# lab-cosmo/torch-pme

Hardware: AMD Instinct MI355X
Metric: atom-steps/sec (energy+forces) (higher is better)
Workload: dtype f32

## Files before the change

### include/mipme.h

```cpp
#ifndef MIPME_H
#define MIPME_H

#include <stdint.h>

#ifdef __cplusplus
extern "C" {
#endif

#define MIPME_VERSION 408

enum { MIPME_F32 = 0, MIPME_F64 = 1 };
enum { MIPME_I64 = 0, MIPME_I32 = 1 };
enum { MIPME_LAGRANGE = 0, MIPME_P3M = 1 };
enum { MIPME_COULOMB = 0, MIPME_INVERSE_POWER_LAW = 1 };

enum {
  MIPME_OK = 0,
  MIPME_EINVAL = -1,
  MIPME_EHIP = -2,
  MIPME_EFFT = -3,
  MIPME_EUNSUPPORTED = -4
};

typedef struct {
// ... 233 lines not shown
  const mipme_potential_t* pot;
  int64_t n_atoms;
  const void* positions;
  const void* charges;
  const void* grad_out;
  const void* G;
  const void* phi_mesh;
  const void* rho_hat;
  const void* rho_dc;
  const void* phi_atoms;
  void* psi_mesh;
  void* psi_hat;
  void* hat_work;
  void* chi_mesh;
  void* dc;
  void* partials;
  void* grad_positions;
  void* grad_charges;
  void* grad_cell;
  void* atom_bins;
  const void* grad_scale;
  const void* mesh_field;
  int64_t kgrid_blocks_ready;
  const void* G_deriv;
} mipme_kspace_backward_args_t;
int mipme_kspace_backward(const mipme_kspace_backward_args_t* args);
int64_t mipme_cellgrad_partials_size(const mipme_mesh_t* mesh, int64_t n_atoms);

int64_t mipme_atom_bins_bytes(const mipme_mesh_t* mesh, int64_t n_atoms, int dtype);
const char* mipme_last_cosched_kernel(void);
int mipme_last_slot_fill(void);
int mipme_last_cell_riders(void);
int mipme_last_gather_pairs(void);
int mipme_plane_spread_parts(const mipme_mesh_t* mesh, int64_t n_atoms, int dtype);

int mipme_profile_enable(int on);
int64_t mipme_profile_report(char* buf, int64_t buflen);

int mipme_slab_forward(void* stream, int dtype, int axis, const mipme_mesh_t* mesh, double prefactor, int64_t n_atoms,
                       const void* positions, const void* charges, void* moments, void* pot);
int mipme_slab_backward(void* stream, int dtype, int axis, const mipme_mesh_t* mesh, double prefactor, int64_t n_atoms,
                        const void* positions, const void* charges, const void* grad_out, void* moments,
                        void* grad_positions, void* grad_charges, void* grad_cell);


int mipme_rspace_forward(void* stream, int dtype, int idx_dtype, int64_t n_pairs, int64_t n_atoms, int n_channels,
                         const void* pairs, const void* dist, const void* charges, const void* pair_mask,
                         int full_list, const mipme_potential_t* pot, int accumulate, void* out_pot);

int mipme_rspace_backward(void* stream, int dtype, int idx_dtype, int64_t n_pairs, int64_t n_atoms, int n_channels,
                          const void* pairs, const void* dist, const void* charges, const void* pair_mask,
                          int full_list, const mipme_potential_t* pot, const void* grad_out, const void* grad_scale,
                          void* grad_dist, void* grad_charges);

int mipme_dot_forward(void* stream, int dtype, int64_t n, const void* a, const void* b, void* scratch ,
                      void* out);
int mipme_dot_backward(void* stream, int dtype, int64_t n, const void* grad, const void* a, const void* b, void* grad_a,
                       void* grad_b);

int mipme_energy_log_push(void* stream, int dtype, int n, const void* src, void* log, void* cursor, int capacity);
int mipme_frames_table_energy_log(int dtype, int n_frames, void* host_table, int64_t host_table_bytes, void* log, void* cursors,
                                  int capacity);

int mipme_scaled_match(void* stream, int dtype, int64_t n, const void* g, const void* q, void* result, void* host_flag);
int64_t mipme_scaled_match_work(int64_t n);
int mipme_scaled_match_wide(void* stream, int dtype, int64_t n, const void* g, const void* q, void* result, void* host_flag,
// ... 357 lines not shown
```

### torch-pme_amd/_lib.py

```python

from __future__ import annotations

import ctypes as C
import os

import torch

_HERE = os.path.dirname(os.path.abspath(__file__))
LIB_PATH = os.environ.get("MIPME_LIB", os.path.join(_HERE, "libmipme.so"))

F32, F64 = 0, 1
I64, I32 = 0, 1
LAGRANGE, P3M = 0, 1
COULOMB, INVERSE_POWER_LAW = 0, 1

EXPORTS = (
    "mipme_last_error", "mipme_version", "mipme_fft_plan_create", "mipme_fft_plan_destroy", "mipme_kfilter_build",
    "mipme_convolve", "mipme_spread", "mipme_gather", "mipme_kspace_forward", "mipme_kspace_backward",
    "mipme_cellgrad_partials_size", "mipme_slab_forward", "mipme_slab_backward", "mipme_rspace_forward",
    "mipme_rspace_backward", "mipme_pair_distance_forward", "mipme_pair_distance_backward",
    "mipme_pair_partials_size", "mipme_topology_workspace_bytes", "mipme_topology_build", "mipme_topology_pack_shifts",
    "mipme_rspace_rows", "mipme_rspace_rows_value_bytes", "mipme_rspace_rows_tabulate", "mipme_rspace_rows_tabulated", "mipme_pair_distance_backward_rows", "mipme_rows_partials_size", "mipme_atom_bins_bytes", "mipme_plane_spread_parts", "mipme_last_cosched_kernel", "mipme_last_slot_fill", "mipme_last_cell_riders", "mipme_last_gather_pairs", "mipme_frames_counter_ints",
    "mipme_profile_enable", "mipme_profile_report", "mipme_dot_forward", "mipme_dot_backward", "mipme_energy_log_push", "mipme_frames_table_energy_log",
    "mipme_nl_workspace_bytes", "mipme_nl_bin", "mipme_nl_count", "mipme_nl_fill", "mipme_nl_stream",
    "mipme_topology_pack_entries", "mipme_sr_rows_fused", "mipme_sr_rows_finalize",
    "mipme_pack_pair_shifts", "mipme_pair_distance_forward_packed", "mipme_fft_plan_xfused", "mipme_fft_plan_kgrid_blocks", "mipme_fft_r2c",
    "mipme_ewald_filter", "mipme_ewald_structure", "mipme_ewald_potential", "mipme_ewald_backward",
    "mipme_frames_table_bytes", "mipme_frames_table_build", "mipme_frames_forward", "mipme_frames_backward",
    "mipme_frames_cell_work", "mipme_frames_table_contract", "mipme_frames_step",
    "mipme_frames_slab_work", "mipme_frames_table_slab", "mipme_frames_slab_step",
    "mipme_frames_table_cells", "mipme_frames_cells", "mipme_frames_cell_geometry",
    "mipme_scaled_match", "mipme_scaled_match_work", "mipme_scaled_match_wide", "mipme_md_supported", "mipme_md_lists_ints", "mipme_md_rebin", "mipme_md_step", "mipme_set_skip_flag", "mipme_energy_select", "mipme_energy_select_sum", "mipme_energy_select_contract",
    "mipme_kfilter_build_deriv", "mipme_cell_tail_work", "mipme_values_equal", "mipme_checksum", "mipme_checksum_words",
    "mipme_spread_jet", "mipme_gather_jet", "mipme_gather_jet3", "mipme_pair_sum", "mipme_pair_sum_rows", "mipme_pair_dot", "mipme_pair_diff", "mipme_pair_scatter",
    "mipme_dipole_rspace_forward", "mipme_dipole_rspace_backward", "mipme_dipole_partials_size", "mipme_dipole_structure",
    "mipme_dipole_field", "mipme_dipole_backward",
    "mipme_spline_eval", "mipme_spline_eval_reciprocal", "mipme_spline_kfilter_build",
    "mipme_combined_sr_eval", "mipme_combined_kfilter_build",
    "mipme_combined_step", "mipme_combined_step_work",
    "mipme_dipole_step", "mipme_dipole_step_work",
    "mipme_ewald_step", "mipme_ewald_step_work",
    "mipme_ewald_batch", "mipme_ewald_batch_work", "mipme_ewald_batch_table_bytes", "mipme_ewald_batch_table_build",
)


class PotentialDesc(C.Structure):
    _fields_ = [
        ("kind", C.c_int32),
        ("exponent", C.c_int32),
        ("smearing", C.c_double),
        ("prefactor", C.c_double),
        ("exclusion_radius", C.c_double),
        ("exclusion_degree", C.c_int32),
        ("_pad", C.c_int32),
    ]
# ... 443 lines not shown
        "mipme_checksum": [vp, vp, i64, vp, vp, vp],
        "mipme_energy_select": [vp, ci, i64, vp, vp, vp, vp, ci, vp, vp],
        "mipme_energy_select_sum": [vp, ci, i64, vp, vp, vp, vp, ci, vp, vp, vp],
        "mipme_energy_select_contract": [vp, ci, i64, vp, vp, vp, vp, ci, vp, vp, vp],
        "mipme_md_rebin": [C.POINTER(MdArgs)],
        "mipme_md_step": [C.POINTER(MdArgs)],
    }
    for name, argtypes in sig.items():
        fn = getattr(lib, name)
        fn.restype = ci
        fn.argtypes = argtypes
    lib.mipme_cellgrad_partials_size.restype = i64
    lib.mipme_cellgrad_partials_size.argtypes = [MP, i64]
    lib.mipme_dipole_partials_size.restype = i64
    lib.mipme_dipole_partials_size.argtypes = [i64, i64]
    lib.mipme_pair_partials_size.restype = i64
    lib.mipme_pair_partials_size.argtypes = [i64]
    lib.mipme_topology_workspace_bytes.restype = i64
    lib.mipme_topology_workspace_bytes.argtypes = [i64]
    lib.mipme_rows_partials_size.restype = i64
    lib.mipme_rows_partials_size.argtypes = [i64]
    lib.mipme_atom_bins_bytes.restype = i64
    lib.mipme_atom_bins_bytes.argtypes = [MP, i64, ci]
    lib.mipme_last_cosched_kernel.restype = C.c_char_p
    lib.mipme_last_cosched_kernel.argtypes = []
    if hasattr(lib, "mipme_last_slot_fill"):
        lib.mipme_last_slot_fill.restype = ci
        lib.mipme_last_slot_fill.argtypes = []
        lib.mipme_last_cell_riders.restype = ci
        lib.mipme_last_cell_riders.argtypes = []
    if hasattr(lib, "mipme_last_gather_pairs"):
        lib.mipme_last_gather_pairs.restype = ci
        lib.mipme_last_gather_pairs.argtypes = []
    lib.mipme_plane_spread_parts.restype = ci
    lib.mipme_plane_spread_parts.argtypes = [MP, i64, ci]
    lib.mipme_frames_counter_ints.restype = i64
    lib.mipme_frames_counter_ints.argtypes = [MP, i64, ci]
    lib.mipme_md_supported.restype = ci
    lib.mipme_md_supported.argtypes = [MP, PP, i64, ci]
    lib.mipme_md_lists_ints.restype = i64
    lib.mipme_md_lists_ints.argtypes = [MP, i64]
    lib.mipme_nl_workspace_bytes.restype = i64
    lib.mipme_nl_workspace_bytes.argtypes = [C.POINTER(NlDesc), i64]
    lib.mipme_rspace_rows_value_bytes.restype = i64
    lib.mipme_rspace_rows_value_bytes.argtypes = [ci, i64]
    lib.mipme_checksum_words.restype = i64
    lib.mipme_checksum_words.argtypes = []
    lib.mipme_cell_tail_work.restype = i64
    lib.mipme_cell_tail_work.argtypes = [vp, MP, i64]
    lib.mipme_fft_plan_xfused.restype = ci
    lib.mipme_fft_plan_xfused.argtypes = [vp]
    lib.mipme_fft_plan_kgrid_blocks.restype = i64
    lib.mipme_fft_plan_kgrid_blocks.argtypes = [vp]
    lib.mipme_frames_cell_work.restype = i64
    lib.mipme_frames_cell_work.argtypes = [MP, i64]
    lib.mipme_combined_step_work.restype = i64
    lib.mipme_combined_step_work.argtypes = [vp, MP, i64, ci]
    lib.mipme_dipole_step_work.restype = i64
    lib.mipme_dipole_step_work.argtypes = [i64, i64, ci]
    lib.mipme_ewald_step_work.restype = i64
    lib.mipme_ewald_step_work.argtypes = [i64, i64, ci]
    lib.mipme_ewald_batch_work.restype = i64
    lib.mipme_ewald_batch_work.argtypes = [ci, vp, vp, ci]
    lib.mipme_ewald_batch_table_bytes.restype = i64
    lib.mipme_ewald_batch_table_bytes.argtypes = [ci, vp, vp, ci]
    lib.mipme_frames_slab_work.restype = i64
# ... 136 lines not shown
```

### torch-pme_amd/csrc/api.hip

```cpp
#include <dlfcn.h>

#include <cmath>
#include <cstring>
#include <map>
#include <string>
#include <vector>

#include "host.h"

namespace mipme {

static thread_local char g_error[512] = "";

static thread_local const char* g_last_cosched = "";
void note_cosched_kernel(const char* name) { g_last_cosched = name ? name : ""; }
static thread_local int g_last_slot_fill = 0;
void note_slot_fill(int rider_atoms) { g_last_slot_fill = rider_atoms; }
static thread_local int g_last_cell_riders = 0;
void note_cell_riders(int n) { g_last_cell_riders = n; }
static thread_local int g_last_gather_pairs = 0;
void note_gather_pairs(int paired) { g_last_gather_pairs = paired; }
void set_error(const char* fmt, ...) {
  va_list ap;
  va_start(ap, fmt);
  vsnprintf(g_error, sizeof(g_error), fmt, ap);
  va_end(ap);
}

struct ProfEntry {
  const char* name;
  hipEvent_t a, b;
  int reps;
};
static constexpr int kProfRepeat = 8;
static bool g_prof_on = false;
static std::vector<ProfEntry> g_prof;

struct Roctx {
  int (*push)(const char*) = nullptr;
  int (*pop)() = nullptr;
  bool on = false;
  Roctx() {
    const char* e = getenv("MIPME_ROCTX");
    if (!e || e[0] == '0') return;
    for (const char* name : {"librocprofiler-sdk-roctx.so", "libroctx64.so"}) {
      if (void* h = dlopen(name, RTLD_NOW | RTLD_GLOBAL)) {
        push = (int (*)(const char*))dlsym(h, "roctxRangePushA");
        pop = (int (*)())dlsym(h, "roctxRangePop");
        if (push && pop) {
          on = true;
          return;
        }
      }
    }
// ... 839 lines not shown
  const ConvCell cc{a.G_deriv, cw.cwave, cw.n_waves, cw.wbuf, cw.rows, int(cw.n_riders), nullptr, nullptr, nullptr, nullptr};
  STAGE(st, "convolve_xfused", convolve_xfused(a.plan, st, a.rho_mesh, a.G, a.hat_work, a.phi_mesh, a.dc, 0, m, a.pot, nullptr,
                                               const_cast<void*>(tail.epart_k), sr_part, n_sr_part, nullptr, a.nan_flag,
                                               a.grad_cell ? &cc : nullptr));
  STAGE(st, "gather+energy+forces",
        live_gather<T>(st, m, a.n_atoms, a.records, a.atom_bins, a.live_lists, a.phi_mesh, a.dc, self_c, bg_c, a.potentials, nullptr,
                       &tail, a.nan_flag));
  if (a.grad_cell)
    STAGE(st, "cell_finalize",
          cell_tail_finalize_impl<T>(st, m, bg_c, 0.5, cw.n_riders, cw.n_bricks, cw.rows, cw.rpart, a.dc,
                                     a.aux_seed ? a.aux_seed : a.grad_seed, a.grad_cell, &tail));
  return MIPME_OK;
}


template <typename T>
static int scaled_match_wide_t(hipStream_t st, int64_t n, const void* g, const void* q, void* result, void* host_flag, void* work) {
  const int64_t nb = (n + 1024 * kMatchRegs - 1) / (1024 * kMatchRegs);
  MIPME_REQUIRE(nb < (int64_t(1) << 24), "mipme_scaled_match_wide: too many values");
  scaled_match_small_kernel<T, true><<<unsigned(nb), 1024, 0, st>>>(n, (const T*)g, (const T*)q, nullptr, nullptr, (double*)work);
  MIPME_LAUNCH_CHECK();
  scaled_match_combine_kernel<T><<<1, 256, 0, st>>>(int(nb), (const double*)work, (T*)result, (int*)host_flag);
  MIPME_LAUNCH_CHECK();
  return MIPME_OK;
}

extern "C" {

const char* mipme_last_error(void) { return g_error; }
const char* mipme_last_cosched_kernel(void) { return g_last_cosched; }
int mipme_last_slot_fill(void) { return g_last_slot_fill; }
int mipme_last_gather_pairs(void) { return g_last_gather_pairs; }
int mipme_last_cell_riders(void) { return g_last_cell_riders; }
int mipme_version(void) { return MIPME_VERSION; }

int mipme_fft_plan_create(int dtype, int nx, int ny, int nz, int batch, mipme_fft_plan** out) {
  return fft_plan_create(dtype, nx, ny, nz, batch, out);
}
int mipme_fft_plan_destroy(mipme_fft_plan* plan) { return fft_plan_destroy(plan); }

int mipme_kfilter_build(void* stream, int dtype, const mipme_mesh_t* mesh, const mipme_potential_t* pot, void* G) {
  int rc = validate_mesh(mesh);
  if (rc) return rc;
  MIPME_REQUIRE(G != nullptr, "G is NULL");
  hipStream_t st = (hipStream_t)stream;
  DT_SWITCH(dtype, kfilter_build_impl<float>(st, mesh, pot, G), kfilter_build_impl<double>(st, mesh, pot, G));
}

int mipme_kfilter_build_deriv(void* stream, int dtype, const mipme_mesh_t* mesh, const mipme_potential_t* pot, void* G_deriv) {
  int rc = validate_mesh(mesh);
  if (rc) return rc;
  MIPME_REQUIRE(G_deriv != nullptr, "G_deriv is NULL");
  hipStream_t st = (hipStream_t)stream;
  DT_SWITCH(dtype, kfilter_deriv_impl<float>(st, mesh, pot, G_deriv), kfilter_deriv_impl<double>(st, mesh, pot, G_deriv));
}

int64_t mipme_cell_tail_work(const mipme_fft_plan* plan, const mipme_mesh_t* mesh, int64_t n_atoms) {
  if (!plan || !mesh || validate_mesh(mesh) || n_atoms < 0) return 0;
  return cell_work_layout(mesh, n_atoms, nullptr).total;
}

int mipme_convolve(mipme_fft_plan* plan, void* stream, const void* mesh_in, const void* G, void* hat_out, void* hat_work,
                   void* mesh_out, void* dc_out) {
  TraceRange _tr("mipme_convolve");
  MIPME_REQUIRE(plan != nullptr, "FFT plan is NULL");
  MIPME_REQUIRE(mesh_in && G && hat_out && hat_work && mesh_out, "NULL buffer passed to mipme_convolve");
// ... 518 lines not shown
```

### torch-pme_amd/csrc/fft_lds.h

```cpp
#pragma once
#include "common.h"

namespace mipme {

template <typename T>
struct Cplx {
  T re, im;
};

__device__ __forceinline__ void unit_root(int j, int n, float& re, float& im) { sincospif(-2.0f * float(j) / float(n), &im, &re); }
__device__ __forceinline__ void unit_root(int j, int n, double& re, double& im) { sincospi(-2.0 * double(j) / double(n), &im, &re); }

template <typename T>
__device__ __forceinline__ Cplx<T> cmul(Cplx<T> a, Cplx<T> w) { return Cplx<T>{a.re * w.re - a.im * w.im, a.re * w.im + a.im * w.re}; }
template <typename T>
__device__ __forceinline__ Cplx<T> cmulc(Cplx<T> a, Cplx<T> w) { return Cplx<T>{a.re * w.re + a.im * w.im, a.im * w.re - a.re * w.im}; }
template <typename T>
__device__ __forceinline__ Cplx<T> cadd(Cplx<T> a, Cplx<T> b) { return Cplx<T>{a.re + b.re, a.im + b.im}; }
template <typename T>
__device__ __forceinline__ Cplx<T> csub(Cplx<T> a, Cplx<T> b) { return Cplx<T>{a.re - b.re, a.im - b.im}; }

template <typename T>
__device__ __forceinline__ Cplx<T> cconj(Cplx<T> a) { return Cplx<T>{a.re, -a.im}; }

// ... 249 lines not shown
}
template <typename T, bool YSTAGE = true>
__device__ __forceinline__ void yz_forward_finish(const YzTile<T>& t, int ny, int nz, int logny, int loglz, Cplx<T>* __restrict__ dst) {
  Cplx<T>* tile = t.tile;
  const Cplx<T>*tw = t.tw, *twr = t.twr;
  const int Lz = t.Lz, RZ = t.RZ, Ltab = t.Ltab;
  const int tid = threadIdx.x, nthr = blockDim.x;
  lds_fft_radix2<T, true, false, MIPME_FFT_ZROWS>(tile, loglz, ny, RZ, 1, tw, Ltab);
  for (int idx = tid; idx < ny * (Lz / 2 + 1); idx += nthr) {
    const int y = idx / (Lz / 2 + 1), k = idx - y * (Lz / 2 + 1);
    Cplx<T>* row = tile + y * RZ;
    const int k2 = Lz - k;
    const Cplx<T> ck = row[k == Lz ? 0 : k], cm = row[k2 == Lz ? 0 : k2];
    const Cplx<T> wk = twr[k], wm = twr[k2];
    auto split = [](Cplx<T> a, Cplx<T> b, Cplx<T> w) {
      const Cplx<T> e{T(0.5) * (a.re + b.re), T(0.5) * (a.im - b.im)};
      const Cplx<T> d{T(0.5) * (a.re - b.re), T(0.5) * (a.im + b.im)};
      const Cplx<T> o{d.im, -d.re};
      return cadd(e, cmul(o, w));
    };
    const Cplx<T> ak = split(ck, cm, wk), am = split(cm, ck, wm);
    row[k] = ak;
    row[k2] = am;
  }
  __syncthreads();
  if constexpr (YSTAGE) lds_fft_radix2<T, false, false, MIPME_FFT_BFAST ? 2 : 0>(tile, logny, RZ, 1, RZ, tw, Ltab);
  for (int idx = tid; idx < ny * RZ; idx += nthr) {
    const int y = idx / RZ, k = idx - y * RZ;
    const int yr = YSTAGE ? int(__brev(unsigned(y)) >> (32 - logny)) : y;
    dst[int64_t(yr) * RZ + k] = tile[idx];
  }
}

template <typename T, bool INVERSE, bool YSTAGE = true>
__device__ __forceinline__ void yz_plane_body(int ny, int nz, int logny, int loglz, const T* __restrict__ real_in,
                                              Cplx<T>* __restrict__ hat, T* __restrict__ real_out, int64_t plane,
                                              char* smem_yz) {
  const YzTile<T> yt = yz_tile_setup<T, YSTAGE>(ny, nz, smem_yz);
  const int Lz = yt.Lz, RZ = yt.RZ, Ltab = yt.Ltab;
  Cplx<T>* tile = yt.tile;
  const Cplx<T>*tw = yt.tw, *twr = yt.twr;
  const int tid = threadIdx.x, nthr = blockDim.x;
  if constexpr (!INVERSE) {
    const T* src = real_in + plane * int64_t(ny) * nz;
    for (int idx = tid; idx < ny * Lz; idx += nthr) {
      const int y = idx / Lz, j = idx - y * Lz;
      const int jr = loglz ? int(__brev(unsigned(j)) >> (32 - loglz)) : 0;
      tile[y * RZ + jr] = reinterpret_cast<const Cplx<T>*>(src)[idx];
    }
    __syncthreads();
    yz_forward_finish<T, YSTAGE>(yt, ny, nz, logny, loglz, hat + plane * int64_t(ny) * RZ);
  } else {
    const Cplx<T>* src = hat + plane * int64_t(ny) * RZ;
    for (int idx = tid; idx < ny * RZ; idx += nthr) {
      const int y = idx / RZ, k = idx - y * RZ;
      const int yr = YSTAGE ? int(__brev(unsigned(y)) >> (32 - logny)) : y;
      tile[yr * RZ + k] = src[idx];
    }
    __syncthreads();
    if constexpr (YSTAGE) lds_fft_radix2<T, true, true, MIPME_FFT_BFAST ? 2 : 0>(tile, logny, RZ, 1, RZ, tw, Ltab);
    for (int idx = tid; idx < ny * (Lz / 2 + 1); idx += nthr) {
      const int y = idx / (Lz / 2 + 1), k = idx - y * (Lz / 2 + 1);
      Cplx<T>* row = tile + y * RZ;
      const int k2 = Lz - k;
      Cplx<T> ak = row[k], am = row[k2];
      if (k == 0) {
        ak.im = T(0);
        am.im = T(0);
      }
      const Cplx<T> wk = twr[k], wm = twr[k2];
      auto merge = [](Cplx<T> a, Cplx<T> b, Cplx<T> w) {
        const Cplx<T> e{a.re + b.re, a.im - b.im};
        const Cplx<T> d{a.re - b.re, a.im + b.im};
        const Cplx<T> dw = cmulc(d, w);
        return Cplx<T>{e.re - dw.im, e.im + dw.re};
      };
      const Cplx<T> ck = merge(ak, am, wk), cm = merge(am, ak, wm);
      if (k < Lz) row[k] = ck;
      if (k2 < Lz && k2 != k) row[k2] = cm;
    }
    __syncthreads();
    lds_fft_radix2<T, false, true, MIPME_FFT_ZROWS>(tile, loglz, ny, RZ, 1, tw, Ltab);
    T* dst = real_out + plane * int64_t(ny) * nz;
    for (int idx = tid; idx < ny * Lz; idx += nthr) {
      const int y = idx / Lz, j = idx - y * Lz;
      const int jr = loglz ? int(__brev(unsigned(j)) >> (32 - loglz)) : 0;
      reinterpret_cast<Cplx<T>*>(dst)[idx] = tile[y * RZ + jr];
    }
  }
}

}
```

### torch-pme_amd/csrc/host.h

```cpp
#pragma once

#include <algorithm>
#include <climits>
#include <cmath>
#include <cstring>

#include "common.h"

namespace mipme {

template <typename T>
constexpr int dtype_of() {
  return sizeof(T) == 4 ? MIPME_F32 : MIPME_F64;
}

#define DT_SWITCH(dtype, CALL_F32, CALL_F64)                    \
  do {                                                          \
    if ((dtype) == MIPME_F32) return CALL_F32;                  \
    if ((dtype) == MIPME_F64) return CALL_F64;                  \
    mipme::set_error("invalid dtype %d", int(dtype));           \
    return MIPME_EINVAL;                                        \
  } while (0)

inline unsigned stride_grid(int64_t n, int block) {
// ... 19 lines not shown
  return MIPME_OK;
}

template <typename T> int spread_impl(hipStream_t st, const mipme_mesh_t* m, int64_t n_atoms, const void* pos, const void* val, double scale,
                                      void* mesh);
template <typename T> int gather_impl(hipStream_t st, const mipme_mesh_t* m, int64_t n_atoms, const void* pos, const void* mesh, void* out);
template <typename T> int gather_epilogue_impl(hipStream_t st, const mipme_mesh_t* m, int64_t n_atoms, const void* pos, const void* mesh,
                                               const void* q, const void* qsum, double self_c, double bg_c, void* out, void* raw,
                                               int accumulate, void* nan_flag);
template <typename T> int gather_grad_impl(hipStream_t st, const mipme_mesh_t* m, int64_t n_atoms, const void* pos, const void* q,
                                           const void* gout, const void* phi, const void* chi, const void* gsum_dc, const void* gscale,
                                           double self_c, double bg_c, void* grad_pos, void* grad_q);

struct FftDims { int dtype, nx, ny, nz, batch; };
int fft_plan_create(int dtype, int nx, int ny, int nz, int batch, mipme_fft_plan** out);
int fft_plan_destroy(mipme_fft_plan* p);
FftDims fft_plan_dims(const mipme_fft_plan* p);
int fft_plan_batch(const mipme_fft_plan* p);
bool fft_plan_xfused(const mipme_fft_plan* p);
int* fft_plan_brick_count(const mipme_fft_plan* p);
int fft_forward(mipme_fft_plan* p, hipStream_t st, const void* in, void* out);
int fft_inverse(mipme_fft_plan* p, hipStream_t st, void* in, void* out);
int64_t xconv_blocks(const mipme_fft_plan* p);
int convolve_xfused(mipme_fft_plan* p, hipStream_t st, const void* mesh_in, const void* G, void* hat, void* mesh_out,
                    void* dc, int64_t G_stride, const mipme_mesh_t* cell_mesh, const mipme_potential_t* cell_pot,
                    void* cell_partials, void* epart, const void* sr_part, int64_t n_sr_part, const RowRideHost* rh,
                    void* err_flag, const ConvCell* cc);
void fft_plan_begin_step(mipme_fft_plan* p);
bool fft_plan_plane_forward_ok(const mipme_fft_plan* p);
bool fft_plan_plane_forward_ok_batched(const mipme_fft_plan* p);
void fft_plan_set_forward_done(mipme_fft_plan* p, bool done, int parts);
void fft_plan_set_forward_ycols(mipme_fft_plan* p, bool pending);
void* fft_plan_hat_parts(mipme_fft_plan* p, hipStream_t st, int n_more);
int fft_plan_tail_scratch(mipme_fft_plan* p, int64_t bytes, void** out);
template <typename T> int kfilter_build_impl(hipStream_t st, const mipme_mesh_t* m, const mipme_potential_t* pot, void* G);
template <typename T> int kfilter_deriv_impl(hipStream_t st, const mipme_mesh_t* m, const mipme_potential_t* pot, void* D);
template <typename T> int apply_filter_impl(hipStream_t st, int64_t Mh, int C, const void* hat, const void* G, void* out, void* dc);
template <typename T> int apply_filter_cellgrad_impl(hipStream_t st, const mipme_mesh_t* m, const mipme_potential_t* pot, const void* psi_hat,
                                                     const void* rho_hat, const void* G, void* out, void* dc, void* partials);
int64_t cellgrad_blocks(const mipme_mesh_t* m);
int64_t cellgrad_scratch_doubles();
template <typename T> int cellgrad_finalize_impl(hipStream_t st, const mipme_mesh_t* m, double bg, int64_t n_atoms, void* partials,
                                                 const void* pos, const void* grad_pos, const void* gout, const void* phi_atoms,
                                                 const void* rho_dc, const void* psi_dc, const void* energy_scale, void* grad_cell,
                                                 int64_t kgrid_blocks, const void* field, const void* q);
template <typename T> int cell_tail_finalize_impl(hipStream_t st, const mipme_mesh_t* m, double bg, double pair_scale, int64_t n_rows,
                                                  int64_t n_bricks, const void* rows, const void* rpart, const void* dc, const void* seed, void* out,
                                                  const GatherTailHost* slab = nullptr);

template <typename T, typename I> int rspace_forward_impl(hipStream_t st, int64_t P, int64_t N, int C, const void* pairs, const void* dist, const void* q,
                                                          const void* mask, int full, const mipme_potential_t* pot, int accumulate, void* out);
template <typename T, typename I> int rspace_backward_impl(hipStream_t st, int64_t P, int64_t N, int C, const void* pairs, const void* dist,
                                                           const void* q, const void* mask, int full, const mipme_potential_t* pot, const void* g,
                                                           const void* gscale, void* grad_d, void* grad_q);
template <typename T, typename I> int distance_forward_impl(hipStream_t st, int64_t P, const void* pairs, const void* pos, const void* cell,
                                                            const void* shifts, void* out);
template <typename T, typename I> int distance_backward_impl(hipStream_t st, int64_t P, int64_t N, const void* pairs, const void* pos, const void* cell,
                                                             const void* shifts, const void* grad_d, void* partials, void* grad_pos, void* grad_cell);
template <typename T> int pack_pair_shifts_impl(hipStream_t st, int64_t P, const void* shifts, void* packed, void* flag);
template <typename T> int distance_forward_packed_impl(hipStream_t st, int64_t P, const void* pairs, const void* packed, const void* pos,
                                                       const void* cell, void* out);
int64_t pair_partials_blocks(int64_t P);

bool bricks_supported(const mipme_mesh_t* m, int dtype);
int64_t bins_bytes(const mipme_mesh_t* m, int64_t N, int dtype);
int plane_bins_capacity(const mipme_mesh_t* m, int64_t N, int dtype);
// ... 130 lines not shown
```

### torch-pme_amd/csrc/kfilter.hip

```cpp
#include <hipfft/hipfft.h>

#include <cmath>
#include <cstdlib>
#include <new>

#include "host.h"
#include "kgrid.h"
#include "kpot.h"
#include "fft_lds.h"
#include "cell_finalize_device.h"
#include "bricks_device.h"

namespace mipme {


template <typename T>
__global__ __launch_bounds__(256) void kfilter_kernel(KGeom g, KPot kp, T* __restrict__ G) {
  const int64_t Mh = int64_t(g.nx) * g.ny * g.nzh;
  const int64_t t = int64_t(blockIdx.x) * blockDim.x + threadIdx.x;
  if (t >= Mh) return;
  double inv, v, dv;
  bool dead;
  const double k2 = kgrid_point(g, t, inv, dead);
  lr_kernel_dev(kp, k2, v, dv);
// ... 379 lines not shown
  MIPME_SKIP_IF_SET(skip);
  extern __shared__ __attribute__((aligned(16))) char smem_yz[];
  if constexpr (INVERSE && YSTAGE) {
    if (blockIdx.x >= n_planes) {
      cell_rider_body<T>(rider, blockIdx.x - n_planes, int(blockDim.x), reinterpret_cast<double*>(smem_yz));
      return;
    }
  }
  yz_plane_body<T, INVERSE, YSTAGE>(ny, nz, logny, loglz, real_in, hat, real_out, blockIdx.x, smem_yz);
}

template <int SCHEME, int N, typename T>
__global__ __launch_bounds__(1024) void yz_planes_slots_kernel(int ny, int nz, int logny, int loglz, Cplx<T>* __restrict__ hat,
                                                             T* __restrict__ real_out, const int* __restrict__ skip,
                                                             unsigned n_planes, CellRider rider, SlotRider slots) {
  MIPME_SKIP_IF_SET(skip);
  extern __shared__ __attribute__((aligned(16))) char smem_yz[];
  if (blockIdx.x >= n_planes + unsigned(rider.n_riders)) {
    slot_rider_body<SCHEME, N, T>(slots, blockIdx.x - n_planes - unsigned(rider.n_riders));
    return;
  }
  if (blockIdx.x >= n_planes) {
    cell_rider_body<T>(rider, blockIdx.x - n_planes, int(blockDim.x), reinterpret_cast<double*>(smem_yz));
    return;
  }
  yz_plane_body<T, true, true>(ny, nz, logny, loglz, nullptr, hat, real_out, blockIdx.x, smem_yz);
}

__device__ __forceinline__ unsigned xcd_tile(unsigned b, unsigned n) {
  const unsigned x = b & 7u, per = n >> 3, rem = n & 7u;
  return x * per + (x < rem ? x : rem) + (b >> 3);
}

template <typename T, bool INVERSE>
__global__ __launch_bounds__(256) void ycols_kernel(int ny, int nzh, int logny, int kzs, int nchunk, Cplx<T>* __restrict__ hat,
                                                   const int* __restrict__ skip) {
  MIPME_SKIP_IF_SET(skip);
  extern __shared__ __attribute__((aligned(16))) char smem_yc[];
  const int KZ = 1 << kzs, KP = KZ + 1;
  Cplx<T>* tile = reinterpret_cast<Cplx<T>*>(smem_yc);
  Cplx<T>* tw = tile + size_t(ny) * KP;
  const int tid = threadIdx.x, nthr = blockDim.x;
  const unsigned tile_id = xcd_tile(blockIdx.x, gridDim.x);
  const int chunk = tile_id % nchunk;
  const int64_t plane = tile_id / nchunk;
  const int kz0 = chunk << kzs, kzn = min(KZ, nzh - kz0);
  for (int j = tid; j < (ny >> 1); j += nthr) unit_root(j, ny, tw[j].re, tw[j].im);
  Cplx<T>* col = hat + plane * int64_t(ny) * nzh + kz0;
  const int n_el = ny << kzs;
  for (int idx = tid; idx < n_el; idx += nthr) {
    const int y = idx >> kzs, z = idx & (KZ - 1);
    const int yt = INVERSE ? int(__brev(unsigned(y)) >> (32 - logny)) : y;
    tile[yt * KP + z] = z < kzn ? col[int64_t(y) * nzh + z] : Cplx<T>{T(0), T(0)};
  }
  __syncthreads();
  lds_fft_radix2<T, INVERSE, INVERSE, MIPME_FFT_BFAST ? 1 : 0>(tile, logny, KZ, 1, KP, tw, ny);
  for (int idx = tid; idx < n_el; idx += nthr) {
    const int y = idx >> kzs, z = idx & (KZ - 1);
    const int ys = INVERSE ? y : int(__brev(unsigned(y)) >> (32 - logny));
    if (z < kzn) col[int64_t(ys) * nzh + z] = tile[y * KP + z];
  }
}

template <typename T>
static int ycols(mipme_fft_plan* p, hipStream_t st, bool inverse, void* hat) {
  const int nzh = p->nz / 2 + 1;
// ... 25 lines not shown
  int loglz = 0;
  while ((1 << loglz) < p->nz / 2) ++loglz;
  const int Lz = p->nz / 2, R = p->split_rows;
  const size_t lds = sizeof(Cplx<T>) * (size_t(R) * (Lz + 1) + size_t(Lz) / 2 + size_t(Lz + 1));
  const unsigned grid = unsigned(int64_t(p->nx) * p->ny * p->batch / R);
  const int work = R * (Lz + 1);
  const int threads = work >= 2048 ? 1024 : (work >= 512 ? 256 : 64);
  if (inverse)
    yz_planes_kernel<T, true, false><<<grid, threads, lds, st>>>(R, p->nz, 0, loglz, nullptr, (Cplx<T>*)hat, (T*)real_out, skip_flag_slot(), grid, CellRider{});
  else
    yz_planes_kernel<T, false, false><<<grid, threads, lds, st>>>(R, p->nz, 0, loglz, (const T*)real_in, (Cplx<T>*)hat, nullptr, skip_flag_slot(), grid, CellRider{});
  MIPME_LAUNCH_CHECK();
  return MIPME_OK;
}

template <typename T>
static int cell_riders_alone(hipStream_t st, const CellRider& r) {
  cell_rider_kernel<T><<<unsigned(r.n_riders), 1024, 0, st>>>(r);
  MIPME_LAUNCH_CHECK();
  return MIPME_OK;
}

static void yz_launch_shape(const mipme_fft_plan* p, size_t real_bytes, int& logny, int& loglz, size_t& lds, int& threads) {
  logny = loglz = 0;
  while ((1 << logny) < p->ny) ++logny;
  while ((1 << loglz) < p->nz / 2) ++loglz;
  const int Lz = p->nz / 2, Ltab = p->ny > Lz ? p->ny : Lz;
  lds = 2 * real_bytes * (size_t(p->ny) * (Lz + 1) + size_t(Ltab) / 2 + size_t(Lz + 1));
  const int work = p->ny * (Lz + 1);
  threads = work >= 2048 ? 1024 : (work >= 512 ? 256 : 64);
}

template <typename T>
static int yz_planes(mipme_fft_plan* p, hipStream_t st, bool inverse, const void* real_in, void* hat, void* real_out,
                     const CellRider* rider = nullptr, const SlotRider* slots = nullptr) {
  MIPME_REQUIRE(!slots || (inverse && !p->split_yz && skip_flag_slot() == nullptr),
                "slot riders need the single-launch inverse planes and a clear skip flag");
  if (p->split_yz) {
    int rc;
    if (!inverse) {
      if ((rc = zrows<T>(p, st, false, real_in, hat, nullptr))) return rc;
      return ycols<T>(p, st, false, hat);
    }
    if (rider && rider->n_riders > 0 && (rc = cell_riders_alone<T>(st, *rider))) return rc;
    if ((rc = ycols<T>(p, st, true, hat))) return rc;
    return zrows<T>(p, st, true, nullptr, hat, real_out);
  }
  int logny = 0, loglz = 0, threads = 0;
  size_t lds = 0;
  yz_launch_shape(p, sizeof(T), logny, loglz, lds, threads);
  const unsigned grid = unsigned(p->nx) * unsigned(p->batch);
  const unsigned n_riders = (inverse && rider) ? unsigned(rider->n_riders) : 0u;
  if (n_riders && lds < sizeof(double) * 16 * kCellRow) lds = sizeof(double) * 16 * kCellRow;
  if (lds > 64 * 1024) {
    static bool raised[2] = {false, false};
    if (!raised[inverse ? 1 : 0]) {
      const void* fn = inverse ? (const void*)yz_planes_kernel<T, true> : (const void*)yz_planes_kernel<T, false>;
      MIPME_CHECK_HIP(hipFuncSetAttribute(fn, hipFuncAttributeMaxDynamicSharedMemorySize, int(kYzMaxLds)));
      raised[inverse ? 1 : 0] = true;
    }
  }
  if (inverse && slots) {
    SlotRider sr = *slots;
    sr.per_rider = threads < kSlotRiderAtoms ? threads : kSlotRiderAtoms;
    const unsigned n_slot_riders = unsigned((sr.n_atoms + sr.per_rider - 1) / sr.per_rider);
    const bool raise = lds > 64 * 1024;
    int slot_rc = MIPME_OK;
    MIPME_DISPATCH_STENCIL_B(sr.scheme, sr.order, (slot_rc = [&]() -> int {
      if (raise) {
        static bool raised_slots = false;
        if (!raised_slots) {
          MIPME_CHECK_HIP(hipFuncSetAttribute((const void*)yz_planes_slots_kernel<S, N, T>, hipFuncAttributeMaxDynamicSharedMemorySize, int(kYzMaxLds)));
          raised_slots = true;
        }
      }
      yz_planes_slots_kernel<S, N, T><<<grid + n_riders + n_slot_riders, threads, lds, st>>>(
          p->ny, p->nz, logny, loglz, (Cplx<T>*)hat, (T*)real_out, skip_flag_slot(), grid, n_riders ? *rider : CellRider{}, sr);
      return MIPME_OK;
    }()));
    if (slot_rc) return slot_rc;
    note_slot_fill(sr.per_rider);
    note_cell_riders(int(n_riders));
  } else if (inverse)
    yz_planes_kernel<T, true><<<grid + n_riders, threads, lds, st>>>(p->ny, p->nz, logny, loglz, nullptr, (Cplx<T>*)hat, (T*)real_out,
                                                                     skip_flag_slot(), grid, n_riders ? *rider : CellRider{});
// ... 328 lines not shown
    rider.cwave = cc->cwave;
    rider.n_waves = int(cc->n_waves);
    rider.epart_k = (const double*)epart;
    rider.n_tiles = int(grid);
    rider.rows = cc->rows;
  }
  const bool forward_done = p->forward_done, forward_ycols = p->forward_ycols;
  p->forward_done = p->forward_ycols = false;
  if (forward_done) {
    if (forward_ycols) {
      int rc = ycols<T>(p, st, false, hat);
      if (rc) return rc;
    }
  } else if (p->own_yz) {
    int rc = yz_planes<T>(p, st, false, mesh_in, hat, nullptr);
    if (rc) return rc;
  } else if (sizeof(T) == 4) {
    MIPME_CHECK_FFT(hipfftExecR2C(p->fwd2d, (hipfftReal*)mesh_in, (hipfftComplex*)hat));
  } else {
    MIPME_CHECK_FFT(hipfftExecD2Z(p->fwd2d, (hipfftDoubleReal*)mesh_in, (hipfftDoubleComplex*)hat));
  }
#define MIPME_XCONV_LAUNCH(MODE)                                                                                              \
  xconv_kernel<T, MODE><<<grid, threads, lds, st>>>(p->nx, p->ny, nzh, log2nx, kzs, nchunk, (Cplx<T>*)hat, (const T*)G,      \
                                                    G_stride, (T*)dc, kg, kp, (double*)cell_partials, (double*)epart,        \
                                                    (const double*)sr_part, int(n_sr_part), skip_flag_slot(), xc)
  if (cell_partials)
    MIPME_XCONV_LAUNCH(1);
  else
    MIPME_XCONV_LAUNCH(0);
#undef MIPME_XCONV_LAUNCH
  MIPME_LAUNCH_CHECK();
  const SlotRider* slots = (cc && cc->slots && cc->slots->n_atoms > 0) ? cc->slots : nullptr;
  MIPME_REQUIRE(!slots || (p->own_yz && p->batch == 1), "slot riders need the plan's own (y,z) plane kernels and a single mesh");
  if (p->own_yz) {
    int rc = yz_planes<T>(p, st, true, nullptr, hat, mesh_out, riders ? &rider : nullptr, slots);
    if (rc) return rc;
  } else {
    if (riders) {
      int rc = cell_riders_alone<T>(st, rider);
      if (rc) return rc;
    }
    if (sizeof(T) == 4)
      MIPME_CHECK_FFT(hipfftExecC2R(p->inv2d, (hipfftComplex*)hat, (hipfftReal*)mesh_out));
    else
      MIPME_CHECK_FFT(hipfftExecZ2D(p->inv2d, (hipfftDoubleComplex*)hat, (hipfftDoubleReal*)mesh_out));
  }
  return MIPME_OK;
}

int convolve_xfused(mipme_fft_plan* p, hipStream_t st, const void* mesh_in, const void* G, void* hat, void* mesh_out,
                    void* dc, int64_t G_stride, const mipme_mesh_t* cell_mesh, const mipme_potential_t* cell_pot,
                    void* cell_partials, void* epart, const void* sr_part, int64_t n_sr_part, const RowRideHost* rh,
                    void* err_flag, const ConvCell* cc) {
  MIPME_REQUIRE(!rh || rh->n_rows <= 0, "row riders on the convolution launches were an experiment of round 2 (tools/r06/pruned_experiments.patch)");
  if (!p->own_yz) {
    MIPME_CHECK_FFT(hipfftSetStream(p->fwd2d, st));
    MIPME_CHECK_FFT(hipfftSetStream(p->inv2d, st));
  }
  if (p->dtype == MIPME_F32)
    return convolve_xfused_t<float>(p, st, mesh_in, G, hat, mesh_out, dc, G_stride, cell_mesh, cell_pot, cell_partials, epart,
                                    sr_part, n_sr_part, cc);
  return convolve_xfused_t<double>(p, st, mesh_in, G, hat, mesh_out, dc, G_stride, cell_mesh, cell_pot, cell_partials, epart,
                                   sr_part, n_sr_part, cc);
}

bool fft_plan_plane_forward_ok(const mipme_fft_plan* p) {
// ... 414 lines not shown
  else
    cell_tail_finalize_kernel<T><<<1, 1024, 0, st>>>(*m, bg, pair_scale, int(n_rows), int(n_bricks), (const double*)rows,
                                                    (const double*)rpart, (const T*)dc, (const T*)seed, (T*)out, SlabCell{});
  MIPME_LAUNCH_CHECK();
  return MIPME_OK;
}

template int kfilter_deriv_impl<float>(hipStream_t, const mipme_mesh_t*, const mipme_potential_t*, void*);
template int kfilter_deriv_impl<double>(hipStream_t, const mipme_mesh_t*, const mipme_potential_t*, void*);
template int cell_tail_finalize_impl<float>(hipStream_t, const mipme_mesh_t*, double, double, int64_t, int64_t, const void*,
                                            const void*, const void*, const void*, void*, const GatherTailHost*);
template int cell_tail_finalize_impl<double>(hipStream_t, const mipme_mesh_t*, double, double, int64_t, int64_t, const void*,
                                             const void*, const void*, const void*, void*, const GatherTailHost*);
template int frames_cell_riders<float>(hipStream_t, const FrameCellRec*, int, int, int, int, int, const double*, int);
template int frames_cell_riders<double>(hipStream_t, const FrameCellRec*, int, int, int, int, int, const double*, int);
template int frames_cell_finalize<float>(hipStream_t, const FrameCellRec*, int);
template int frames_cell_finalize<double>(hipStream_t, const FrameCellRec*, int);
template int kfilter_build_impl<float>(hipStream_t, const mipme_mesh_t*, const mipme_potential_t*, void*);
template int kfilter_build_impl<double>(hipStream_t, const mipme_mesh_t*, const mipme_potential_t*, void*);
template int apply_filter_impl<float>(hipStream_t, int64_t, int, const void*, const void*, void*, void*);
template int apply_filter_impl<double>(hipStream_t, int64_t, int, const void*, const void*, void*, void*);
template int apply_filter_cellgrad_impl<float>(hipStream_t, const mipme_mesh_t*, const mipme_potential_t*, const void*,
                                               const void*, const void*, void*, void*, void*);
template int apply_filter_cellgrad_impl<double>(hipStream_t, const mipme_mesh_t*, const mipme_potential_t*,
                                                const void*, const void*, const void*, void*, void*, void*);
template int cellgrad_finalize_impl<float>(hipStream_t, const mipme_mesh_t*, double, int64_t, void*, const void*,
                                           const void*, const void*, const void*, const void*, const void*, const void*,
                                           void*, int64_t, const void*, const void*);
template int cellgrad_finalize_impl<double>(hipStream_t, const mipme_mesh_t*, double, int64_t, void*, const void*,
                                            const void*, const void*, const void*, const void*, const void*, const void*,
                                            void*, int64_t, const void*, const void*);

}
```

Measured before the change: 612.3 million.

## Split inverse y-z plane FFT across multiple workgroups per plane

Adds a split variant of the inverse y/z plane kernel. It decomposes each x-plane's y-FFT by a first radix-2 or radix-4 stage done while loading from global memory, so each of S workgroups handles ny/S rows of one plane. The aim is more workgroups on small meshes where nx planes alone underfill the GPU. The split factor is chosen automatically when nx*S stays at or below 128 workgroups, and an environment variable can override it. Each workgroup reads S strided rows from global memory and does extra twiddle work, and the change also adds optional timeline probes and a query for the split factor.

Result: faster. 622.1 million (median of 6 runs) (+1.6%).

```diff
diff --git a/include/mipme.h b/include/mipme.h
--- a/include/mipme.h
+++ b/include/mipme.h
@@ -289,6 +289,7 @@
 int mipme_last_slot_fill(void);
 int mipme_last_cell_riders(void);
 int mipme_last_gather_pairs(void);
+int mipme_last_inverse_split(void);
 int mipme_plane_spread_parts(const mipme_mesh_t* mesh, int64_t n_atoms, int dtype);
 
 int mipme_profile_enable(int on);
diff --git a/torch-pme_amd/_lib.py b/torch-pme_amd/_lib.py
--- a/torch-pme_amd/_lib.py
+++ b/torch-pme_amd/_lib.py
@@ -20,7 +20,7 @@
     "mipme_cellgrad_partials_size", "mipme_slab_forward", "mipme_slab_backward", "mipme_rspace_forward",
     "mipme_rspace_backward", "mipme_pair_distance_forward", "mipme_pair_distance_backward",
     "mipme_pair_partials_size", "mipme_topology_workspace_bytes", "mipme_topology_build", "mipme_topology_pack_shifts",
-    "mipme_rspace_rows", "mipme_rspace_rows_value_bytes", "mipme_rspace_rows_tabulate", "mipme_rspace_rows_tabulated", "mipme_pair_distance_backward_rows", "mipme_rows_partials_size", "mipme_atom_bins_bytes", "mipme_plane_spread_parts", "mipme_last_cosched_kernel", "mipme_last_slot_fill", "mipme_last_cell_riders", "mipme_last_gather_pairs", "mipme_frames_counter_ints",
+    "mipme_rspace_rows", "mipme_rspace_rows_value_bytes", "mipme_rspace_rows_tabulate", "mipme_rspace_rows_tabulated", "mipme_pair_distance_backward_rows", "mipme_rows_partials_size", "mipme_atom_bins_bytes", "mipme_plane_spread_parts", "mipme_last_cosched_kernel", "mipme_last_slot_fill", "mipme_last_cell_riders", "mipme_last_gather_pairs", "mipme_last_inverse_split", "mipme_frames_counter_ints",
     "mipme_profile_enable", "mipme_profile_report", "mipme_dot_forward", "mipme_dot_backward", "mipme_energy_log_push", "mipme_frames_table_energy_log",
     "mipme_nl_workspace_bytes", "mipme_nl_bin", "mipme_nl_count", "mipme_nl_fill", "mipme_nl_stream",
     "mipme_topology_pack_entries", "mipme_sr_rows_fused", "mipme_sr_rows_finalize",
@@ -530,6 +530,9 @@
     if hasattr(lib, "mipme_last_gather_pairs"):
         lib.mipme_last_gather_pairs.restype = ci
         lib.mipme_last_gather_pairs.argtypes = []
+    if hasattr(lib, "mipme_last_inverse_split"):
+        lib.mipme_last_inverse_split.restype = ci
+        lib.mipme_last_inverse_split.argtypes = []
     lib.mipme_plane_spread_parts.restype = ci
     lib.mipme_plane_spread_parts.argtypes = [MP, i64, ci]
     lib.mipme_frames_counter_ints.restype = i64
diff --git a/torch-pme_amd/csrc/api.hip b/torch-pme_amd/csrc/api.hip
--- a/torch-pme_amd/csrc/api.hip
+++ b/torch-pme_amd/csrc/api.hip
@@ -20,6 +20,8 @@
 void note_cell_riders(int n) { g_last_cell_riders = n; }
 static thread_local int g_last_gather_pairs = 0;
 void note_gather_pairs(int paired) { g_last_gather_pairs = paired; }
+static thread_local int g_last_inverse_split = 1;
+void note_inverse_split(int split) { g_last_inverse_split = split; }
 void set_error(const char* fmt, ...) {
   va_list ap;
   va_start(ap, fmt);
@@ -925,6 +927,7 @@
 int mipme_last_slot_fill(void) { return g_last_slot_fill; }
 int mipme_last_gather_pairs(void) { return g_last_gather_pairs; }
 int mipme_last_cell_riders(void) { return g_last_cell_riders; }
+int mipme_last_inverse_split(void) { return g_last_inverse_split; }
 int mipme_version(void) { return MIPME_VERSION; }
 
 int mipme_fft_plan_create(int dtype, int nx, int ny, int nz, int batch, mipme_fft_plan** out) {
diff --git a/torch-pme_amd/csrc/fft_lds.h b/torch-pme_amd/csrc/fft_lds.h
--- a/torch-pme_amd/csrc/fft_lds.h
+++ b/torch-pme_amd/csrc/fft_lds.h
@@ -305,6 +305,16 @@
   }
 }
 
+#if defined(MIPME_WG_TIMELINE) && MIPME_WG_TIMELINE == 2
+static __device__ long long g_yz_phase[8 * 1024];
+#define MIPME_YZ_PHASE(wg, k)                                                                                             \
+  do {                                                                                                                    \
+    if (threadIdx.x == 0 && (wg) < 1024) g_yz_phase[(wg) * 8 + (k)] = (long long)__builtin_amdgcn_s_memrealtime();         \
+  } while (0)
+#else
+#define MIPME_YZ_PHASE(wg, k)
+#endif
+
 template <typename T, bool INVERSE, bool YSTAGE = true>
 __device__ __forceinline__ void yz_plane_body(int ny, int nz, int logny, int loglz, const T* __restrict__ real_in,
                                               Cplx<T>* __restrict__ hat, T* __restrict__ real_out, int64_t plane,
@@ -324,6 +334,7 @@
     __syncthreads();
     yz_forward_finish<T, YSTAGE>(yt, ny, nz, logny, loglz, hat + plane * int64_t(ny) * RZ);
   } else {
+    MIPME_YZ_PHASE(plane, 0);
     const Cplx<T>* src = hat + plane * int64_t(ny) * RZ;
     for (int idx = tid; idx < ny * RZ; idx += nthr) {
       const int y = idx / RZ, k = idx - y * RZ;
@@ -331,7 +342,9 @@
       tile[yr * RZ + k] = src[idx];
     }
     __syncthreads();
+    MIPME_YZ_PHASE(plane, 1);
     if constexpr (YSTAGE) lds_fft_radix2<T, true, true, MIPME_FFT_BFAST ? 2 : 0>(tile, logny, RZ, 1, RZ, tw, Ltab);
+    MIPME_YZ_PHASE(plane, 2);
     for (int idx = tid; idx < ny * (Lz / 2 + 1); idx += nthr) {
       const int y = idx / (Lz / 2 + 1), k = idx - y * (Lz / 2 + 1);
       Cplx<T>* row = tile + y * RZ;
@@ -354,13 +367,111 @@
     }
     __syncthreads();
     lds_fft_radix2<T, false, true, MIPME_FFT_ZROWS>(tile, loglz, ny, RZ, 1, tw, Ltab);
+    MIPME_YZ_PHASE(plane, 3);
     T* dst = real_out + plane * int64_t(ny) * nz;
     for (int idx = tid; idx < ny * Lz; idx += nthr) {
       const int y = idx / Lz, j = idx - y * Lz;
       const int jr = loglz ? int(__brev(unsigned(j)) >> (32 - loglz)) : 0;
       reinterpret_cast<Cplx<T>*>(dst)[idx] = tile[y * RZ + jr];
     }
-  }
-}
-
-}
+#if defined(MIPME_WG_TIMELINE) && MIPME_WG_TIMELINE == 2
+    __syncthreads();
+    MIPME_YZ_PHASE(plane, 4);
+#endif
+  }
+}
+
+#ifndef MIPME_INV_SPLIT_NARROW
+#define MIPME_INV_SPLIT_NARROW 0
+#endif
+template <typename T, int S>
+__device__ __forceinline__ void yz_inverse_split_body(int ny, int nz, int logny, int loglz, const Cplx<T>* __restrict__ hat,
+                                                      T* __restrict__ real_out, int64_t plane, int h, unsigned wg, char* smem_yz) {
+  static_assert(S == 2 || S == 4, "radix of the split stage");
+  constexpr int LOGS = S == 2 ? 1 : 2;
+  const int M = ny >> LOGS, logM = logny - LOGS;
+  MIPME_YZ_PHASE(wg, 0);
+  const YzTile<T> yt = yz_tile_setup<T, true>(M, nz, smem_yz);
+  const int Lz = yt.Lz, RZ = yt.RZ, Ltab = yt.Ltab;
+  Cplx<T>* tile = yt.tile;
+  const Cplx<T>*tw = yt.tw, *twr = yt.twr;
+  const int tid = threadIdx.x, nthr = blockDim.x;
+  const Cplx<T>* src = hat + plane * int64_t(ny) * RZ;
+  const int items = M * RZ, jstride = M * RZ;
+  const T s2 = (h & 1) ? T(-1) : T(1);
+  const Cplx<T> ih{T(h == 0 ? 1 : (h == 2 ? -1 : 0)), T(h == 1 ? 1 : (h == 3 ? -1 : 0))};
+  constexpr int U = MIPME_INV_SPLIT_NARROW ? 3 : 4 / S;
+  for (int base = tid; base < items; base += U * nthr) {
+    Cplx<T> x[U][S];
+#pragma unroll
+    for (int u = 0; u < U; ++u) {
+      const int idx = base + u * nthr;
+      const Cplx<T>* q = src + (idx < items ? idx : 0);
+#pragma unroll
+      for (int j = 0; j < S; ++j) x[u][j] = q[j * jstride];
+    }
+    Cplx<T> w[U];
+    int slot[U];
+#pragma unroll
+    for (int u = 0; u < U; ++u) {
+      const int idx = base + u * nthr;
+      const int k = idx / RZ, kz = idx - k * RZ;
+      unit_root(idx < items ? k * h : 0, ny, w[u].re, w[u].im);
+      slot[u] = int(__brev(unsigned(k)) >> (32 - logM)) * RZ + kz;
+    }
+#pragma unroll
+    for (int u = 0; u < U; ++u) {
+      const int idx = base + u * nthr;
+      if (idx < items) {
+        Cplx<T> a;
+        if constexpr (S == 2) {
+          a = Cplx<T>{x[u][0].re + s2 * x[u][1].re, x[u][0].im + s2 * x[u][1].im};
+        } else {
+          const Cplx<T> e{x[u][0].re + s2 * x[u][2].re, x[u][0].im + s2 * x[u][2].im};
+          const Cplx<T> o{x[u][1].re + s2 * x[u][3].re, x[u][1].im + s2 * x[u][3].im};
+          a = cadd(e, cmul(o, ih));
+        }
+        tile[slot[u]] = cmulc(a, w[u]);
+      }
+    }
+  }
+  __syncthreads();
+  MIPME_YZ_PHASE(wg, 1);
+  lds_fft_radix2<T, true, true, MIPME_FFT_BFAST ? 2 : 0>(tile, logM, RZ, 1, RZ, tw, Ltab);
+  MIPME_YZ_PHASE(wg, 2);
+  for (int idx = tid; idx < M * (Lz / 2 + 1); idx += nthr) {
+    const int y = idx / (Lz / 2 + 1), k = idx - y * (Lz / 2 + 1);
+    Cplx<T>* row = tile + y * RZ;
+    const int k2 = Lz - k;
+    Cplx<T> ak = row[k], am = row[k2];
+    if (k == 0) {
+      ak.im = T(0);
+      am.im = T(0);
+    }
+    const Cplx<T> wk = twr[k], wm = twr[k2];
+    auto merge = [](Cplx<T> a, Cplx<T> b, Cplx<T> w) {
+      const Cplx<T> e{a.re + b.re, a.im - b.im};
+      const Cplx<T> d{a.re - b.re, a.im + b.im};
+      const Cplx<T> dw = cmulc(d, w);
+      return Cplx<T>{e.re - dw.im, e.im + dw.re};
+    };
+    const Cplx<T> ck = merge(ak, am, wk), cm = merge(am, ak, wm);
+    if (k < Lz) row[k] = ck;
+    if (k2 < Lz && k2 != k) row[k2] = cm;
+  }
+  __syncthreads();
+  lds_fft_radix2<T, false, true, MIPME_FFT_ZROWS>(tile, loglz, M, RZ, 1, tw, Ltab);
+  MIPME_YZ_PHASE(wg, 3);
+  Cplx<T>* dst = reinterpret_cast<Cplx<T>*>(real_out + plane * int64_t(ny) * nz);
+  for (int idx = tid; idx < M * Lz; idx += nthr) {
+    const int m = idx / Lz, j = idx - m * Lz;
+    const int jr = loglz ? int(__brev(unsigned(j)) >> (32 - loglz)) : 0;
+    dst[(S * m + h) * Lz + j] = tile[m * RZ + jr];
+  }
+#if defined(MIPME_WG_TIMELINE) && MIPME_WG_TIMELINE == 2
+  __syncthreads();
+  MIPME_YZ_PHASE(wg, 4);
+#endif
+}
+
+}
diff --git a/torch-pme_amd/csrc/host.h b/torch-pme_amd/csrc/host.h
--- a/torch-pme_amd/csrc/host.h
+++ b/torch-pme_amd/csrc/host.h
@@ -75,6 +75,18 @@
 void fft_plan_set_forward_done(mipme_fft_plan* p, bool done, int parts);
 void fft_plan_set_forward_ycols(mipme_fft_plan* p, bool pending);
 void* fft_plan_hat_parts(mipme_fft_plan* p, hipStream_t st, int n_more);
+inline int inverse_plane_split_setting() {
+  const char* e = getenv("MIPME_INV_PLANE_SPLIT");
+  const int s = e ? atoi(e) : 0;
+  return (s == 1 || s == 2 || s == 4) ? s : 0;
+}
+static constexpr int kInvPlaneSplitMaxWorkgroups = 128;
+inline int inverse_plane_split_auto(int nx, int ny) {
+  for (int s = 4; s > 1; s >>= 1)
+    if (s * nx <= kInvPlaneSplitMaxWorkgroups && ny >= 4 * s) return s;
+  return 1;
+}
+void note_inverse_split(int split);
 int fft_plan_tail_scratch(mipme_fft_plan* p, int64_t bytes, void** out);
 template <typename T> int kfilter_build_impl(hipStream_t st, const mipme_mesh_t* m, const mipme_potential_t* pot, void* G);
 template <typename T> int kfilter_deriv_impl(hipStream_t st, const mipme_mesh_t* m, const mipme_potential_t* pot, void* D);
diff --git a/torch-pme_amd/csrc/kfilter.hip b/torch-pme_amd/csrc/kfilter.hip
--- a/torch-pme_amd/csrc/kfilter.hip
+++ b/torch-pme_amd/csrc/kfilter.hip
@@ -435,6 +435,39 @@
   return x * per + (x < rem ? x : rem) + (b >> 3);
 }
 
+template <typename T, int S>
+__global__ __launch_bounds__(1024) void yz_planes_split_kernel(int ny, int nz, int logny, int loglz, const Cplx<T>* __restrict__ hat,
+                                                                 T* __restrict__ real_out, const int* __restrict__ skip,
+                                                                 unsigned n_items, CellRider rider) {
+  MIPME_SKIP_IF_SET(skip);
+  extern __shared__ __attribute__((aligned(16))) char smem_yz[];
+  if (blockIdx.x >= n_items) {
+    cell_rider_body<T>(rider, blockIdx.x - n_items, int(blockDim.x), reinterpret_cast<double*>(smem_yz));
+    return;
+  }
+  const unsigned item = xcd_tile(blockIdx.x, n_items);
+  yz_inverse_split_body<T, S>(ny, nz, logny, loglz, hat, real_out, item / S, int(item % S), item, smem_yz);
+}
+
+template <int SCHEME, int N, typename T, int S>
+__global__ __launch_bounds__(1024) void yz_planes_slots_split_kernel(int ny, int nz, int logny, int loglz,
+                                                                       const Cplx<T>* __restrict__ hat, T* __restrict__ real_out,
+                                                                       const int* __restrict__ skip, unsigned n_items,
+                                                                       CellRider rider, SlotRider slots) {
+  MIPME_SKIP_IF_SET(skip);
+  extern __shared__ __attribute__((aligned(16))) char smem_yz[];
+  if (blockIdx.x >= n_items + unsigned(rider.n_riders)) {
+    slot_rider_body<SCHEME, N, T>(slots, blockIdx.x - n_items - unsigned(rider.n_riders));
+    return;
+  }
+  if (blockIdx.x >= n_items) {
+    cell_rider_body<T>(rider, blockIdx.x - n_items, int(blockDim.x), reinterpret_cast<double*>(smem_yz));
+    return;
+  }
+  const unsigned item = xcd_tile(blockIdx.x, n_items);
+  yz_inverse_split_body<T, S>(ny, nz, logny, loglz, hat, real_out, item / S, int(item % S), item, smem_yz);
+}
+
 template <typename T, bool INVERSE>
 __global__ __launch_bounds__(256) void ycols_kernel(int ny, int nzh, int logny, int kzs, int nchunk, Cplx<T>* __restrict__ hat,
                                                    const int* __restrict__ skip) {
@@ -526,6 +559,49 @@
 }
 
 template <typename T>
+static int inverse_split_for(const mipme_fft_plan* p, size_t lds1, const void* hat, const void* real_out) {
+  int s = inverse_plane_split_setting();
+  if (s == 0) s = inverse_plane_split_auto(p->nx, p->ny);
+  if (s == 1 || p->batch != 1 || p->ny < 4 * s || lds1 > 64 * 1024) return 1;
+  const char *h0 = static_cast<const char*>(hat), *r0 = static_cast<const char*>(real_out);
+  const size_t planes = size_t(p->nx) * p->ny;
+  const char *h1 = h0 + planes * (p->nz / 2 + 1) * 2 * sizeof(T), *r1 = r0 + planes * p->nz * sizeof(T);
+  return (h0 < r1 && r0 < h1) ? 1 : s;
+}
+
+template <typename T, int SPLIT>
+static int yz_planes_split(mipme_fft_plan* p, hipStream_t st, const void* hat, void* real_out, int logny, int loglz, int threads,
+                           const CellRider* rider, const SlotRider* slots) {
+#if MIPME_INV_SPLIT_NARROW
+  threads = threads / SPLIT > 64 ? threads / SPLIT : 64;
+#endif
+  const int Lz = p->nz / 2, M = p->ny / SPLIT, Ltab = M > Lz ? M : Lz;
+  size_t lds = sizeof(Cplx<T>) * (size_t(M) * (Lz + 1) + size_t(Ltab) / 2 + size_t(Lz + 1));
+  const unsigned n_items = unsigned(p->nx) * unsigned(SPLIT);
+  const unsigned n_riders = rider ? unsigned(rider->n_riders) : 0u;
+  if (n_riders && lds < sizeof(double) * 16 * kCellRow) lds = sizeof(double) * 16 * kCellRow;
+  if (slots) {
+    SlotRider sr = *slots;
+    sr.per_rider = threads < kSlotRiderAtoms ? threads : kSlotRiderAtoms;
+    const unsigned n_slot_riders = unsigned((sr.n_atoms + sr.per_rider - 1) / sr.per_rider);
+    int slot_rc = MIPME_OK;
+    MIPME_DISPATCH_STENCIL_B(sr.scheme, sr.order, (slot_rc = [&]() -> int {
+      yz_planes_slots_split_kernel<S, N, T, SPLIT><<<n_items + n_riders + n_slot_riders, threads, lds, st>>>(
+          p->ny, p->nz, logny, loglz, (const Cplx<T>*)hat, (T*)real_out, skip_flag_slot(), n_items, n_riders ? *rider : CellRider{}, sr);
+      return MIPME_OK;
+    }()));
+    if (slot_rc) return slot_rc;
+    note_slot_fill(sr.per_rider);
+    note_cell_riders(int(n_riders));
+  } else {
+    yz_planes_split_kernel<T, SPLIT><<<n_items + n_riders, threads, lds, st>>>(p->ny, p->nz, logny, loglz, (const Cplx<T>*)hat, (T*)real_out,
+                                                                          skip_flag_slot(), n_items, n_riders ? *rider : CellRider{});
+  }
+  MIPME_LAUNCH_CHECK();
+  return MIPME_OK;
+}
+
+template <typename T>
 static int yz_planes(mipme_fft_plan* p, hipStream_t st, bool inverse, const void* real_in, void* hat, void* real_out,
                      const CellRider* rider = nullptr, const SlotRider* slots = nullptr) {
   MIPME_REQUIRE(!slots || (inverse && !p->split_yz && skip_flag_slot() == nullptr),
@@ -545,6 +621,12 @@
   yz_launch_shape(p, sizeof(T), logny, loglz, lds, threads);
   const unsigned grid = unsigned(p->nx) * unsigned(p->batch);
   const unsigned n_riders = (inverse && rider) ? unsigned(rider->n_riders) : 0u;
+  if (inverse) {
+    const int split = inverse_split_for<T>(p, lds, hat, real_out);
+    note_inverse_split(split);
+    if (split == 2) return yz_planes_split<T, 2>(p, st, hat, real_out, logny, loglz, threads, n_riders ? rider : nullptr, slots);
+    if (split == 4) return yz_planes_split<T, 4>(p, st, hat, real_out, logny, loglz, threads, n_riders ? rider : nullptr, slots);
+  }
   if (n_riders && lds < sizeof(double) * 16 * kCellRow) lds = sizeof(double) * 16 * kCellRow;
   if (lds > 64 * 1024) {
     static bool raised[2] = {false, false};
@@ -939,6 +1021,7 @@
   MIPME_LAUNCH_CHECK();
   const SlotRider* slots = (cc && cc->slots && cc->slots->n_atoms > 0) ? cc->slots : nullptr;
   MIPME_REQUIRE(!slots || (p->own_yz && p->batch == 1), "slot riders need the plan's own (y,z) plane kernels and a single mesh");
+  note_inverse_split(1);
   if (p->own_yz) {
     int rc = yz_planes<T>(p, st, true, nullptr, hat, mesh_out, riders ? &rider : nullptr, slots);
     if (rc) return rc;
@@ -1419,3 +1502,9 @@
                                             void*, int64_t, const void*, const void*);
 
 }
+
+#if defined(MIPME_WG_TIMELINE) && MIPME_WG_TIMELINE == 2
+extern "C" int mipme_debug_yz_phase(void* out, int n_words) {
+  return (int)hipMemcpyFromSymbol(out, HIP_SYMBOL(mipme::g_yz_phase), size_t(n_words) * 8);
+}
+#endif
```
